# robertteleng/aria-slam

Measured on AMD Instinct MI355X. Metric: frames/s ORB extract+BF-match, 640x480 @2000 kp, higher is better.
Workload: dtype u8

## Files before the change

aria_slam_amd/csrc/orb_kernels.h:

```cpp
#pragma once
#include <hip/hip_runtime.h>
#include <hip/hip_ext.h>

#include <cstdint>
#include <vector>

#include "aria_orb_hip.h"
#include "orb_plan.h"

namespace aria {

struct FrameSrc {
    const uint8_t* img;
    int64_t frame_stride;
    int row_stride;
    int aligned4;
    int aligned16;
};

struct DeviceScratch {
    uint8_t* raw;
    uint8_t* blur;
    uint32_t* cand;
    int* cand_cnt;
    uint4* sel;
    int* sel_cnt;
    uint32_t* tab;
    int* pyr_bands;
    int* err;
    int* ovf;
    int2* ovf_items;
    unsigned long long* ovf_keys;
    long long ovf_keys_cap;
    uint4* osel;
    int osel_cap;
};

enum { STAGE_RESIZE = 0, STAGE_FAST_BLUR = 1, STAGE_SELECT = 2, STAGE_DESCRIBE = 3, STAGE_COUNT = 4 };
struct LaunchEvents { hipEvent_t start, stop; int stage; int launches; };
struct Profiler {
    bool enabled = false;
    unsigned stage_mask = ~0u;
    bool open = false;
    std::vector<LaunchEvents> pending;
    std::vector<hipEvent_t> pool;
    double ms[STAGE_COUNT] = {0, 0, 0, 0};
    int64_t launches[STAGE_COUNT] = {0, 0, 0, 0};
    int64_t frames = 0;
    LaunchEvents cur{};
    hipEvent_t get();
    void begin(int stage, hipStream_t st);
    void count() { cur.launches++; }
    void end(hipStream_t st);
    void collect();
    void release();
};

struct EnvConfig {
    int ablate;
    int level_streams;
    int stamp_level;
    int sel_stamps;
    int band_trim;
    int band_xcd_map;
    int select_bitonic;
    int desc_stamps;
    int fast_blur_impl;
    int fuse_resize;
    int pyr_impl;
    int rs_impl;
    int band_budget_kb, band_qpct0, band_qstep;
    int batch_stream;
};
const EnvConfig& env_config();

struct LaunchCtx {
    int device = -1;
    int schedule = 0;
    int* hdr = nullptr;
    const uint8_t* host_img = nullptr;
    hipEvent_t stage_event[4] = {};
    bool stage_events_armed = false;
    bool last_blur_q4 = false;
    const char* last_fast_blur = "";
    hipStream_t side[kLevels] = {};
    hipEvent_t ev_fork = nullptr, ev_join[kLevels] = {}, ev_lvl[kLevels] = {};
    unsigned long long* d_band_stamps = nullptr;
    unsigned long long* d_sel_stamps = nullptr;
    unsigned long long* d_desc_stamps = nullptr;
    int init(int device);
    void release();
};

#define ARIA_LAUNCH(prof, kernel, grid, block, lds, st, ...)                       \
    do {                                                                           \
        if ((prof) && (prof)->open) (prof)->count();                               \
        hipLaunchKernelGGL(kernel, grid, block, lds, st, __VA_ARGS__);             \
    } while (0)

void launch_fast_blur_band(const Plan& P, const FrameSrc& S, const DeviceScratch& D, int n_frames, hipStream_t st,
                           Profiler* prof, bool fuse_resize, LaunchCtx& ctx);
void launch_band2(const Plan& P, const FrameSrc& S, const DeviceScratch& D, int n_frames, hipStream_t st, Profiler* prof,
                  bool fuse_resize, LaunchCtx& ctx);
int band2_set_attributes();
void launch_fast_blur_stream(const Plan& P, const FrameSrc& S, const DeviceScratch& D, int n_frames, hipStream_t st,
                             Profiler* prof, LaunchCtx& ctx);
bool stream_eligible(const Plan& P, const FrameSrc& S);
int stream_set_attributes();
int blur_tail_start(int tie_mode, int w);
int band_set_attributes();
int band_init_ctx(LaunchCtx& ctx);
int band_side_streams(LaunchCtx& ctx);

struct BandAll { int first[kLevels + 1]; int qcap[kLevels]; int xcd_map; int lpr[kLevels]; };
bool launch_pyramid_fused(const Plan& P, const FrameSrc& S, const DeviceScratch& D, int n_frames, hipStream_t st, Profiler* prof,
                          int* clr_a = nullptr, int n_a = 0, int* clr_b = nullptr, int n_b = 0,
                          const uint8_t* src_alt = nullptr, uint8_t* copy_dst = nullptr);
bool pyramid_fused_available(const Plan& P);
bool latency_zero_copy(const Plan& P, const LaunchCtx& ctx, const Profiler* prof);
void launch_pyramid_level(const Plan& P, const FrameSrc& S, const DeviceScratch& D, int n_frames, hipStream_t st, Profiler* prof, int l);
void launch_pyramid_and_band_latency(const Plan& P, const FrameSrc& S, const DeviceScratch& D, int n_frames, hipStream_t st,
                                     Profiler* prof, LaunchCtx& ctx);
void launch_pyramid_pass(const Plan& P, const FrameSrc& S, const DeviceScratch& D, int n_frames, hipStream_t st, Profiler* prof);
int pyramid_set_attributes();
void launch_fast_blur_tile(const Plan& P, const FrameSrc& S, const DeviceScratch& D, int n_frames, hipStream_t st, Profiler* prof);

void launch_extract_chunk(const Plan& P, const FrameSrc& S, const DeviceScratch& D, int n_frames,
                          aria_keypoint* d_kps, uint8_t* d_desc, int* d_counts, int kp_cap, hipStream_t st,
                          Profiler* prof, LaunchCtx& ctx);

}
```

aria_slam_amd/csrc/orb_kernels.hip:

```cpp
#include <hip/hip_runtime.h>

#include <cfloat>
#include <cstdint>
#include <cstdlib>

#include "common.h"
#include "orb_device.h"
#include "orb_kernels.h"

namespace aria {

struct PatternLaneMajor { uint32_t w[16][16]; };
constexpr PatternLaneMajor make_pattern_lane_major() {
    constexpr int src[1024] = {
#include "orb_pattern_31.inc"
    };
    PatternLaneMajor p{};
    for (int l = 0; l < 16; l++)
        for (int it = 0; it < 16; it++) {
            const int t = 16 * it + l;
            p.w[l][it] = ((uint32_t)(src[4 * t] & 0xFF)) | ((uint32_t)(src[4 * t + 1] & 0xFF) << 8) |
                         ((uint32_t)(src[4 * t + 2] & 0xFF) << 16) | ((uint32_t)(src[4 * t + 3] & 0xFF) << 24);
        }
    return p;
// ... 470 lines not shown
                uint32_t u = __float_as_uint(r);
                u = (u & 0x80000000u) ? ~u : (u | 0x80000000u);
                key = ((unsigned long long)(~u) << 32) | ((uint32_t)y << 16) | (uint32_t)x;
            }
            const unsigned long long m = __ballot(keep);
            if (m) {
                const int lane = tid & 63, leader = __ffsll((long long)m) - 1;
                int base = 0;
                if (lane == leader) base = atomicAdd(&s_misc[1], __popcll(m));
                base = __shfl(base, leader);
                if (keep) ovf_st(&K[base + __popcll(m & ((1ull << lane) - 1ull))], key);
            }
        }
        for (long long i = n1 + tid; i < np; i += 256) ovf_st(&K[i], ~0ull);
        __syncthreads();
        for (long long k = 2; k <= np; k <<= 1)
            for (long long j = k >> 1; j > 0; j >>= 1) {
                for (long long t = tid; t < (np >> 1); t += 256) {
                    const long long a = ((t & ~(j - 1)) << 1) | (t & (j - 1)), b = a | j;
                    const unsigned long long xa = ovf_ld(&K[a]), xb = ovf_ld(&K[b]);
                    if ((xa > xb) == ((a & k) == 0)) { ovf_st(&K[a], xb); ovf_st(&K[b], xa); }
                }
                __syncthreads();
            }
        int n2 = n1;
        if (n1 > q) {
            const uint32_t cut = (uint32_t)(ovf_ld(&K[q - 1]) >> 32);
            for (int i = q + tid; i < n1; i += 256)
                if ((uint32_t)(ovf_ld(&K[i]) >> 32) == cut) atomicAdd(&s_misc[2], 1);
            __syncthreads();
            n2 = q + s_misc[2];
        }
        const int extra = max(n2 - g.sel_cap, 0), extra4 = (extra + 3) & ~3;
        if (tid == 0) {
            int ob = 0;
            if (extra4 > 0) {
                ob = atomicAdd(&ovf[1], extra4);
                if (ob + extra4 > osel_cap) { atomicOr(err, ERRBIT_SEL_OVERFLOW); ob = -1; }
            }
            s_misc[4] = ob;
        }
        __syncthreads();
        const int ob = s_misc[4];
        if (ob < 0) n2 = g.sel_cap;
        uint4* out = sel + (int64_t)frame * P.sel_frame_entries + g.sel_off;
        const uint32_t tag = (uint32_t)frame | ((uint32_t)l << 24);
        for (int i = tid; i < n2; i += 256) {
            const unsigned long long kk = ovf_ld(&K[i]);
            uint32_t u = ~(uint32_t)(kk >> 32);
            u = (u & 0x80000000u) ? (u & 0x7FFFFFFFu) : ~u;
            const uint4 rec = make_uint4((uint32_t)kk, u, (uint32_t)i, tag);
            if (i < g.sel_cap) out[i] = rec;
            else osel[ob + (i - g.sel_cap)] = rec;
        }
        if (ob >= 0)
            for (int i = extra + tid; i < extra4; i += 256) osel[ob + i] = make_uint4(0u, 0u, 0xFFFFFFFFu, tag);
        if (tid == 0) sel_cnt[frame * kLevels + l] = n2;
    }
}

__global__ __launch_bounds__(256) void k_select_ovf(Plan P, FrameSrc S, const uint8_t* __restrict__ raw,
                                                    const uint32_t* __restrict__ cand, const int* __restrict__ cand_cnt,
                                                    uint4* __restrict__ sel, int* __restrict__ sel_cnt, int* __restrict__ err,
                                                    int* __restrict__ ovf, const int2* __restrict__ ovf_items,
                                                    unsigned long long* __restrict__ keys, long long keys_cap,
                                                    uint4* __restrict__ osel, int osel_cap) {
    __shared__ int s_hist[256];
    __shared__ __attribute__((aligned(8))) int s_misc[8];
    const int n_items = min(ovf[0], kOvfItems);
    for (int it = blockIdx.x; it < n_items; it += gridDim.x)
        select_ovf_item(P, S, raw, cand, cand_cnt, sel, sel_cnt, err, ovf, keys, keys_cap, osel, osel_cap, ovf_items[it].x,
                        ovf_items[it].y, s_hist, s_misc);
}

__device__ __forceinline__ float fast_atan2_deg(float y, float x) {
    const float p1 = 0.9997878412794807f * (float)(180 / 3.1415926535897932384626433832795);
    const float p3 = -0.3258083974640975f * (float)(180 / 3.1415926535897932384626433832795);
    const float p5 = 0.1555786518463281f * (float)(180 / 3.1415926535897932384626433832795);
    const float p7 = -0.04432655554792128f * (float)(180 / 3.1415926535897932384626433832795);
    const float ax = fabsf(x), ay = fabsf(y);
    float a, c, c2;
    if (ax >= ay) {
        c = ay / (ax + (float)DBL_EPSILON);
        c2 = c * c;
        a = (((p7 * c2 + p5) * c2 + p3) * c2 + p1) * c;
    } else {
        c = ax / (ay + (float)DBL_EPSILON);
        c2 = c * c;
        a = 90.f - (((p7 * c2 + p5) * c2 + p3) * c2 + p1) * c;
    }
    if (x < 0) a = 180.f - a;
    if (y < 0) a = 360.f - a;
    return a;
}

__device__ __forceinline__ void det_sincos(double x, double& s, double& c) {
    const double invpio2 = 6.36619772367581382433e-01;
    const double pio2_hi = 1.57079632673412561417e+00;
    const double pio2_lo = 6.07710050650619224932e-11;
    const double S1 = -1.66666666666666324348e-01, S2 = 8.33333333332248946124e-03,
                 S3 = -1.98412698298579493134e-04, S4 = 2.75573137070700676789e-06,
                 S5 = -2.50507602534068634195e-08, S6 = 1.58969099521155010221e-10;
    const double C1 = 4.16666666666666019037e-02, C2 = -1.38888888888741095749e-03,
                 C3 = 2.48015872894767294178e-05, C4 = -2.75573143513906633035e-07,
                 C5 = 2.08757232129817482790e-09, C6 = -1.13596475577881948265e-11;
    const double fn = floor(x * invpio2 + 0.5);
    const double r = (x - fn * pio2_hi) - fn * pio2_lo;
    const double z = r * r;
    const double sp = S2 + z * (S3 + z * (S4 + z * (S5 + z * S6)));
    const double sn = r + (z * r) * (S1 + z * sp);
    const double cp = z * (C1 + z * (C2 + z * (C3 + z * (C4 + z * (C5 + z * C6)))));
    const double cs = 1.0 - (0.5 * z - z * cp);
    const int qd = (int)fn & 3;
    s = (qd == 0) ? sn : (qd == 1) ? cs : (qd == 2) ? -sn : -cs;
    c = (qd == 0) ? cs : (qd == 1) ? -sn : (qd == 2) ? -cs : sn;
}

__device__ __forceinline__ int wave_sum(int v) {
    v += __builtin_amdgcn_update_dpp(0, v, 0xB1, 0xF, 0xF, true);
    v += __builtin_amdgcn_update_dpp(0, v, 0x4E, 0xF, 0xF, true);
    v += __builtin_amdgcn_update_dpp(0, v, 0x141, 0xF, 0xF, true);
    v += __builtin_amdgcn_update_dpp(0, v, 0x140, 0xF, 0xF, true);
    v += __builtin_amdgcn_update_dpp(0, v, 0x142, 0xA, 0xF, false);
    v += __builtin_amdgcn_update_dpp(0, v, 0x143, 0xC, 0xF, false);
    return __builtin_amdgcn_readlane(v, 63);
}

constexpr int kDescR = 18;
constexpr int kDescRows = 2 * kDescR + 1;
constexpr int kDescPitch = 64;
constexpr int kDescWaves = 2;
constexpr int kDescKp = 4 * kDescWaves;
constexpr int kIcPitch = 48;
struct __attribute__((packed, aligned(4))) DwordQuad { uint32_t a, b, c, d; };

__device__ __forceinline__ int row8_sum(int v) {
    v += __builtin_amdgcn_update_dpp(0, v, 0xB1, 0xF, 0xF, true);
    v += __builtin_amdgcn_update_dpp(0, v, 0x4E, 0xF, 0xF, true);
    v += __builtin_amdgcn_update_dpp(0, v, 0x141, 0xF, 0xF, true);
    return v;
}

__device__ __forceinline__ int row16_sum(int v) {
    v += __builtin_amdgcn_update_dpp(0, v, 0xB1, 0xF, 0xF, true);
    v += __builtin_amdgcn_update_dpp(0, v, 0x4E, 0xF, 0xF, true);
    v += __builtin_amdgcn_update_dpp(0, v, 0x141, 0xF, 0xF, true);
    v += __builtin_amdgcn_update_dpp(0, v, 0x140, 0xF, 0xF, true);
    return v;
}

constexpr int kDescArenaBlocks = 32;
constexpr int kDescQ = 10;
constexpr int kDescPitchQ = 4 * kDescQ;
template <int MODE, bool Q4>
__global__ __launch_bounds__(64 * kDescWaves) void k_describe(Plan P, FrameSrc S, const uint8_t* __restrict__ raw,
                                                  const uint8_t* __restrict__ blur, const uint4* __restrict__ sel,
                                                  const int* __restrict__ sel_cnt, aria_keypoint* __restrict__ kps,
                                                  uint8_t* __restrict__ desc, int* __restrict__ counts, int kp_cap,
                                                  int* __restrict__ err, int n_frames, int blocks_per_frame,
                                                  unsigned long long* __restrict__ stamps,
                                                  const uint4* __restrict__ osel, const int* __restrict__ ovf, int osel_cap) {
#define DSTAMP(k) do { if (stamps && (threadIdx.x & 63) == 0) stamps[((size_t)blockIdx.x * kDescWaves + (threadIdx.x >> 6)) * 8 + (k)] = __builtin_amdgcn_s_memtime(); } while (0)
    DSTAMP(0);
    constexpr int kPatchBytes = Q4 ? kDescPitchQ * kDescPitchQ : kDescRows * kDescPitch;
    static_assert(kPatchBytes >= 31 * kIcPitch && kPatchBytes % 16 == 0, "the raw window shares the allocation");
    __shared__ __attribute__((aligned(16))) uint8_t s_patch[kDescKp][kPatchBytes];
    uint8_t (*s_raw)[kPatchBytes] = s_patch;
    const int lane = threadIdx.x & 63, wv = threadIdx.x >> 6;
    const int grp = lane >> 4, l16 = lane & 15;
    const int n_regular = MODE == 2 ? (int)gridDim.x - kDescArenaBlocks : (int)gridDim.x;
    auto describe_block = [&](const int blk_in, const bool ARENA) {
    const int blk = __builtin_amdgcn_readfirstlane(blk_in);
    int frame, l = 0, base = 0, nk;
    uint4 sv;
    if (!ARENA) {
        const int xcd = blk & 7, j = blk >> 3;
        frame = __builtin_amdgcn_readfirstlane((j / blocks_per_frame) * 8 + xcd);
        if (frame >= n_frames) return;
        const int jm = __builtin_amdgcn_readfirstlane(j % blocks_per_frame);
        const int slot0 = __builtin_amdgcn_readfirstlane(jm * kDescKp + wv * 4);
        const int* cnt = sel_cnt + frame * kLevels;
        int total = 0;
#pragma unroll
        for (int i = 0; i < kLevels; i++) {
            const int ci = cnt[i];
            if (i > 0 && slot0 >= P.lv[i].sel_off) { l = i; base = total; }
            total += ci;
        }
        if (slot0 == 0 && lane == 0) {
            counts[frame] = min(total, kp_cap);
            if (total > kp_cap) atomicMax(err + 2, total);
        }
        if (slot0 >= P.sel_frame_entries) return;
        l = __builtin_amdgcn_readfirstlane(l);
        base = __builtin_amdgcn_readfirstlane(base);
        const int i0 = slot0 - P.lv[l].sel_off;
        nk = min(4, min(cnt[l], P.lv[l].sel_cap) - i0);
        if (nk <= 0) return;
        sv = sel[(int64_t)frame * P.sel_frame_entries + slot0 + min(grp, nk - 1)];
    } else {
        const int e0 = blk * kDescKp + wv * 4;
        if (e0 >= min(ovf[1], osel_cap)) return;
        const uint4 mine = osel[e0 + grp];
        const unsigned long long vm = __ballot(mine.z != 0xFFFFFFFFu && l16 == 0);
        nk = __popcll(vm);
        if (nk <= 0) return;
        const uint32_t tag = (uint32_t)__builtin_amdgcn_readfirstlane((int)mine.w);
        frame = (int)(tag & 0xFFFFFFu);
        l = (int)(tag >> 24);
        const int* cnt = sel_cnt + frame * kLevels;
        for (int i = 0; i < l; i++) base += cnt[i];
        sv = osel[e0 + min(grp, nk - 1)];
    }
    const LevelGeom g = P.lv[l];
    const bool valid = grp < nk;
    const int oidx = base + (int)sv.z;
    const bool fits = oidx < kp_cap;
    if (valid && !fits && l16 == 0) atomicOr(err, ERRBIT_KPCAP);
    const int x = sv.x & 0xFFFF, y = sv.x >> 16;
    if (stamps) { asm volatile("s_waitcnt vmcnt(0)" ::: "memory"); }
    DSTAMP(1);

    uint32_t icm[16];
#pragma unroll
    for (int k = 0; k < 16; k += 4) {
        const uint4 m4 = *reinterpret_cast<const uint4*>(&kIcMask.m[l16][k]);
        icm[k] = m4.x; icm[k + 1] = m4.y; icm[k + 2] = m4.z; icm[k + 3] = m4.w;
    }
    int pat[16];
#pragma unroll
    for (int it = 0; it < 16; it += 4) {
        const uint4 p4 = *reinterpret_cast<const uint4*>(&kPattern31.w[l16][it]);
        pat[it] = (int)p4.x; pat[it + 1] = (int)p4.y; pat[it + 2] = (int)p4.z; pat[it + 3] = (int)p4.w;
    }

    const uint8_t* bl = blur + (int64_t)frame * P.blur_frame_bytes + g.blur_off;
    const int xs = Q4 ? ((x - kDescR) & ~3) : ((x - kDescR) & ~15);
    const int ys = Q4 ? ((y - kDescR) & ~3) : (y - kDescR);
    constexpr int kPv = Q4 ? 7 : 10;
    DwordQuad pv[kPv];
    int pq[kPv], pc[kPv];
    if constexpr (Q4) {
        const int64_t qp = (int64_t)g.pitch * 4;
        const uint8_t* gp = bl + (int64_t)(ys >> 2) * qp + (xs >> 2) * 16;
#pragma unroll
        for (int k = 0; k < kPv; k++) {
            const int p = min(16 * k + l16, kDescQ * kDescQ - 1);
            pq[k] = (p * 205) >> 11;
            pc[k] = p - kDescQ * pq[k];
            pv[k] = *reinterpret_cast<const DwordQuad*>(gp + pq[k] * qp + pc[k] * 16);
        }
    } else {
        const int r4 = l16 >> 2, c4 = l16 & 3;
        const int64_t p64 = g.pitch;
        const uint8_t* gp = bl + (int64_t)(y - kDescR) * p64 + xs + 16 * c4;
#pragma unroll
        for (int k = 0; k < 10; k++) {
            const int row = (4 * k + 4 <= kDescRows) ? 4 * k + r4 : min(4 * k + r4, kDescRows - 1);
            pv[k] = *reinterpret_cast<const DwordQuad*>(gp + row * p64);
        }
        (void)pq; (void)pc;
    }
    const int rr = l16 / 3, cc = l16 - 3 * rr;
    int pitch;
    const uint8_t* img = raw_level_ptr(P, S, raw, frame, l, pitch);
    const bool raw_dword = __builtin_amdgcn_readfirstlane((l > 0) || S.aligned4) != 0;
    const bool raw_a16 = __builtin_amdgcn_readfirstlane((l > 0) || S.aligned16) != 0;
    const int xr = raw_a16 ? ((x - kHalfPatch) & ~15) : ((x - kHalfPatch) & ~3);
    {
        uint8_t* sr = s_raw[wv * 4 + grp] + 16 * cc;
        const int64_t p64 = pitch;
        const uint8_t* gp = img + (int64_t)(y - kHalfPatch) * p64 + xr + 16 * cc;
        DwordQuad rv[7];
        if (raw_dword) {
#pragma unroll
            for (int k = 0; k < 7; k++) {
                const int row = (5 * k + 5 < 31) ? 5 * k + rr : min(5 * k + rr, 30);
                rv[k] = *reinterpret_cast<const DwordQuad*>(gp + row * p64);
            }
        } else {
#pragma unroll
            for (int k = 0; k < 7; k++) {
                const int row = (5 * k + 5 < 31) ? 5 * k + rr : min(5 * k + rr, 30);
                const uint8_t* q = gp + row * p64;
                rv[k].a = (uint32_t)q[0] | ((uint32_t)q[1] << 8) | ((uint32_t)q[2] << 16) | ((uint32_t)q[3] << 24);
                rv[k].b = (uint32_t)q[4] | ((uint32_t)q[5] << 8) | ((uint32_t)q[6] << 16) | ((uint32_t)q[7] << 24);
                rv[k].c = (uint32_t)q[8] | ((uint32_t)q[9] << 8) | ((uint32_t)q[10] << 16) | ((uint32_t)q[11] << 24);
                rv[k].d = (uint32_t)q[12] | ((uint32_t)q[13] << 8) | ((uint32_t)q[14] << 16) | ((uint32_t)q[15] << 24);
            }
        }
#pragma unroll
        for (int k = 0; k < 7; k++) {
            const int row = (5 * k + 5 < 31) ? 5 * k + rr : min(5 * k + rr, 30);
            *reinterpret_cast<uint4*>(sr + row * kIcPitch) = make_uint4(rv[k].a, rv[k].b, rv[k].c, rv[k].d);
        }
    }
    if (stamps) { asm volatile("s_waitcnt vmcnt(0) lgkmcnt(0)" ::: "memory"); }
    DSTAMP(2);
    __builtin_amdgcn_wave_barrier();

    const int sh = (x - xr) - kHalfPatch;
    const int hp = l16 >> 3, jj = l16 & 7;
    const uint8_t* rbase = s_raw[wv * 4 + grp] + 4 * jj + (sh & ~3);
    const uint32_t wu = 0x04030201u + 0x04040404u * (uint32_t)jj;
    uint32_t acc_u = 0, acc_v = 0, acc_s = 0;
#pragma unroll
    for (int k = 0; k < 16; k++) {
        const int r = min(2 * k + hp, 30);
        const uint32_t lo = *reinterpret_cast<const uint32_t*>(rbase + r * kIcPitch);
        const uint32_t hi = *reinterpret_cast<const uint32_t*>(rbase + r * kIcPitch + 4);
        const uint32_t pix = __builtin_amdgcn_alignbyte(hi, lo, sh) & icm[k];
        acc_u = __builtin_amdgcn_udot4(pix, wu, acc_u, false);
        acc_v = __builtin_amdgcn_udot4(pix, 0x01010101u * (uint32_t)(2 * k + 1), acc_v, false);
        acc_s = __builtin_amdgcn_sad_u8(pix, 0u, acc_s);
    }
    const int sum_u = row16_sum((int)acc_u), sum_v = row16_sum((int)acc_v);
    const int s_half = row8_sum((int)acc_s);
    const int s_othr = __builtin_amdgcn_update_dpp(0, s_half, 0x140, 0xF, 0xF, true);
    const int s_all = s_half + s_othr;
    const int s_hp1 = hp ? s_half : s_othr;
    const int m10 = sum_u - 16 * s_all;
    const int m01 = sum_v + s_hp1 - 16 * s_all;
    const float angle = fast_atan2_deg((float)m01, (float)m10);
    DSTAMP(3);

    float ang = angle;
    ang *= (float)(3.1415926535897932384626433832795 / 180.f);
    double sd, cd;
    det_sincos((double)ang, sd, cd);
    const float a = (float)cd, b = (float)sd;
    __builtin_amdgcn_wave_barrier();
    constexpr int kPitchL = Q4 ? kDescPitchQ : kDescPitch;
    if constexpr (Q4) {
        uint8_t* sp = s_patch[wv * 4 + grp];
#pragma unroll
        for (int k = 0; k < kPv; k++) {
            uint32_t* d = reinterpret_cast<uint32_t*>(sp + (4 * pq[k]) * kPitchL + 4 * pc[k]);
            d[0] = pv[k].a; d[kPitchL / 4] = pv[k].b; d[2 * kPitchL / 4] = pv[k].c; d[3 * kPitchL / 4] = pv[k].d;
        }
    } else {
        const int r4 = l16 >> 2, c4 = l16 & 3;
        uint8_t* sp = s_patch[wv * 4 + grp] + 16 * c4;
#pragma unroll
        for (int k = 0; k < 10; k++) {
            const int row = (4 * k + 4 <= kDescRows) ? 4 * k + r4 : min(4 * k + r4, kDescRows - 1);
            *reinterpret_cast<uint4*>(sp + row * kDescPitch) = make_uint4(pv[k].a, pv[k].b, pv[k].c, pv[k].d);
        }
    }
    const uint8_t* bc = s_patch[wv * 4 + grp] + (y - ys) * kPitchL + (x - xs);
    __builtin_amdgcn_wave_barrier();
    typedef float f2 __attribute__((ext_vector_type(2)));
    const f2 aa = {a, a}, bb = {b, b}, nbb = {-b, -b};
    const f2 magic = {12582912.0f, 12582912.0f};
    constexpr uint32_t kMagicBits = 0x4B400000u;
    const uint8_t* bc0 = bc - (size_t)(0x400000u * (uint32_t)kPitchL + kMagicBits);
    DSTAMP(4);
    uint32_t mine = 0;
#pragma unroll
    for (int it = 0; it < 16; it++) {
        const float px0 = (float)(signed char)(pat[it] & 0xFF), py0 = (float)(signed char)((pat[it] >> 8) & 0xFF);
        const float px1 = (float)(signed char)((pat[it] >> 16) & 0xFF), py1 = (float)(signed char)((pat[it] >> 24) & 0xFF);
        const f2 PX = {px0, px1}, PY = {py0, py1};
        const f2 fx = PX * aa + PY * nbb + magic;
        const f2 fy = PX * bb + PY * aa + magic;
        const uint32_t o0 = __umul24(__float_as_uint(fy.x), kPitchL) + __float_as_uint(fx.x);
        const uint32_t o1 = __umul24(__float_as_uint(fy.y), kPitchL) + __float_as_uint(fx.y);
        const int t0 = bc0[o0];
        const int t1 = bc0[o1];
        const unsigned long long m = __ballot(t0 < t1);
        if (__builtin_amdgcn_inverse_ballot_w64(0x0001000100010001ull << it)) mine = (uint32_t)(m >> (16 * grp)) & 0xFFFFu;
    }
    DSTAMP(5);
    if (valid && fits) {
        const int64_t orow = (int64_t)frame * kp_cap + oidx;
        *reinterpret_cast<uint16_t*>(desc + orow * 32 + 2 * l16) = (uint16_t)mine;
        if (l16 == 0) {
            aria_keypoint k;
            k.x = (float)x * g.scale;
            k.y = (float)y * g.scale;
            k.size = kPatchSize * g.scale;
            k.angle = angle;
            k.response = __uint_as_float(sv.y);
            k.octave = l;
            kps[orow] = k;
        }
    }
    };
    if constexpr (MODE == 0) {
        describe_block((int)blockIdx.x, false);
    } else if constexpr (MODE == 1) {
        const int n_blk = (min(ovf[1], osel_cap) + kDescKp - 1) / kDescKp;
        for (int blk = blockIdx.x; blk < n_blk; blk += gridDim.x) describe_block(blk, true);
    } else {
        if ((int)blockIdx.x < n_regular) {
            describe_block((int)blockIdx.x, false);
        } else {
            const int n_blk = (min(ovf[1], osel_cap) + kDescKp - 1) / kDescKp;
            for (int blk = (int)blockIdx.x - n_regular; blk < n_blk; blk += kDescArenaBlocks) describe_block(blk, true);
        }
    }
    DSTAMP(6);
#undef DSTAMP
}

static int env_int(const char* name, int dflt) { const char* e = aria_getenv(name); return e ? atoi(e) : dflt; }
static bool env_is(const char* name, char c) { const char* e = aria_getenv(name); return e && e[0] == c; }

const EnvConfig& env_config() {
    static const EnvConfig cfg = [] {
        EnvConfig c{};
        c.ablate = env_int("ARIA_ABLATE", 0);
        c.level_streams = env_is("ARIA_LEVEL_STREAMS", '1') ? 1 : 0;
        c.stamp_level = env_int("ARIA_STAMPS", -1);
        c.sel_stamps = env_is("ARIA_SEL_STAMPS", '1') ? 1 : 0;
        c.select_bitonic = env_is("ARIA_SELECT_SORT", 'b') ? 1 : 0;
        c.band_xcd_map = env_is("ARIA_BAND_XCD_MAP", '0') ? 0 : 1;
        c.band_trim = env_is("ARIA_BAND_TRIM", '0') ? 0 : 1;
        c.desc_stamps = env_is("ARIA_DESC_STAMPS", '1') ? 1 : 0;
        c.fast_blur_impl = env_is("ARIA_FAST_BLUR_IMPL", 't') ? 0 : env_is("ARIA_FAST_BLUR_IMPL", 'm') ? 1 : 2;
        c.pyr_impl = env_is("ARIA_PYRAMID_IMPL", 'f') ? 1 : 0;
        c.rs_impl = env_is("ARIA_RESIZE_IMPL", 'd') ? 0 : env_is("ARIA_RESIZE_IMPL", 'l') ? 1 : 2;
        c.fuse_resize = (c.fast_blur_impl != 0 && !env_is("ARIA_RESIZE_FUSE", '0') && !aria_getenv("ARIA_RESIZE_IMPL") &&
                         !aria_getenv("ARIA_PYRAMID_IMPL") && !c.level_streams) ? 1 : 0;
        c.band_budget_kb = env_int("ARIA_BAND_BUDGET_KB", 0);
        c.band_qpct0 = env_int("ARIA_BAND_QPCT0", -1);
        c.band_qstep = env_int("ARIA_BAND_QPCT_STEP", -1);
        c.batch_stream = (c.fast_blur_impl == 2 && !env_is("ARIA_FAST_BLUR_IMPL", 'b') && c.fuse_resize && c.stamp_level < 0) ? 1 : 0;
        return c;
    }();
    return cfg;
}

hipEvent_t Profiler::get() {
    if (!pool.empty()) { hipEvent_t e = pool.back(); pool.pop_back(); return e; }
    hipEvent_t e = nullptr;
    if (hipEventCreate(&e) != hipSuccess) return nullptr;
    return e;
}
void Profiler::begin(int stage, hipStream_t st) {
    open = enabled && ((stage_mask >> stage) & 1u);
    if (!open) return;
    cur = LaunchEvents{get(), get(), stage, 0};
    hipStreamSynchronize(st);
    hipEventRecord(cur.start, st);
}
void Profiler::end(hipStream_t st) {
    if (!open) return;
    open = false;
    hipEventRecord(cur.stop, st);
    hipStreamSynchronize(st);
    pending.push_back(cur);
}
void Profiler::collect() {
    for (LaunchEvents& le : pending) {
        float t = 0.f;
        if (hipEventElapsedTime(&t, le.start, le.stop) == hipSuccess) ms[le.stage] += t;
        launches[le.stage] += le.launches;
        pool.push_back(le.start);
        pool.push_back(le.stop);
    }
    pending.clear();
}
void Profiler::release() {
    collect();
    for (hipEvent_t e : pool) hipEventDestroy(e);
    pool.clear();
}

int LaunchCtx::init(int dev) {
    device = dev;
    const EnvConfig& E = env_config();
    ARIA_HIP(hipFuncSetAttribute(reinterpret_cast<const void*>(k_select<false, 256>), hipFuncAttributeMaxDynamicSharedMemorySize,
                                 (int)(sizeof(unsigned long long) * kSortCapMax)));
    ARIA_HIP(hipFuncSetAttribute(reinterpret_cast<const void*>(k_select<true, 256>), hipFuncAttributeMaxDynamicSharedMemorySize,
                                 (int)(sizeof(unsigned long long) * kSortCapMax)));
    if (int prc = pyramid_set_attributes(); prc != ARIA_OK) return prc;
    int rc = band_set_attributes();
    if (rc != ARIA_OK) return rc;
#ifdef ARIA_VARIANTS
    rc = band2_set_attributes();
    if (rc != ARIA_OK) return rc;
#endif
    rc = stream_set_attributes();
    if (rc != ARIA_OK) return rc;
    rc = band_init_ctx(*this);
    if (rc != ARIA_OK) return rc;
    if (E.sel_stamps) ARIA_HIP(hipMalloc(&d_sel_stamps, sizeof(unsigned long long) * 8 * kLevels * 4096));
    if (E.desc_stamps) ARIA_HIP(hipMalloc(&d_desc_stamps, sizeof(unsigned long long) * 8 * (1u << 22)));
    return ARIA_OK;
}

void LaunchCtx::release() {
    for (int l = 0; l < kLevels; l++) {
        if (side[l]) hipStreamDestroy(side[l]);
        if (ev_join[l]) hipEventDestroy(ev_join[l]);
        if (ev_lvl[l]) hipEventDestroy(ev_lvl[l]);
        side[l] = nullptr; ev_join[l] = nullptr; ev_lvl[l] = nullptr;
    }
    if (ev_fork) hipEventDestroy(ev_fork);
    ev_fork = nullptr;
    hipFree(d_band_stamps); hipFree(d_sel_stamps); hipFree(d_desc_stamps);
    d_band_stamps = d_sel_stamps = d_desc_stamps = nullptr;
}

static bool latency_schedule(const LaunchCtx& ctx, const Profiler* prof) {
    return ctx.schedule == 1 && ctx.ev_fork != nullptr && env_config().fast_blur_impl == 2 && !(prof && prof->enabled);
}

bool latency_zero_copy(const Plan& P, const LaunchCtx& ctx, const Profiler* prof) {
    static const bool off = [] { const char* e = aria_getenv("ARIA_ZERO_COPY"); return !(e && e[0] == '1'); }();
    const char* f = aria_getenv("ARIA_LATENCY_FORK");
    return !off && !(f && f[0] == '1') && ctx.host_img != nullptr && latency_schedule(ctx, prof) && pyramid_fused_available(P);
}

void launch_extract_chunk(const Plan& P, const FrameSrc& S, const DeviceScratch& D, int n_frames,
                          aria_keypoint* d_kps, uint8_t* d_desc, int* d_counts, int kp_cap, hipStream_t st,
                          Profiler* prof, LaunchCtx& ctx) {
    const EnvConfig& E = env_config();
    if (prof && prof->enabled) prof->frames += n_frames;

    const bool latency = latency_schedule(ctx, prof);
    const bool fuse_resize = E.fuse_resize != 0 && !latency;
    ctx.last_blur_q4 = false;
    if (!latency) {
        hipMemsetAsync(D.ovf, 0, sizeof(int) * (4 + kLevels * (size_t)n_frames), st);
        if (ctx.hdr) hipMemsetAsync(ctx.hdr, 0, 64, st);
    }
    if (latency) {
        ctx.last_fast_blur = "k_fast_blur_band";
        launch_pyramid_and_band_latency(P, S, D, n_frames, st, prof, ctx);
    } else {
#ifdef ARIA_VARIANTS
    if (!fuse_resize) {
        if (prof) prof->begin(STAGE_RESIZE, st);
        launch_pyramid_pass(P, S, D, n_frames, st, prof);
        if (prof) prof->end(st);
    }
#endif

    if (prof) prof->begin(STAGE_FAST_BLUR, st);
    if (E.batch_stream && fuse_resize && stream_eligible(P, S)) {
        ctx.last_fast_blur = "k_fast_blur_stream";
        ctx.last_blur_q4 = true;
        launch_fast_blur_stream(P, S, D, n_frames, st, prof, ctx);
#ifdef ARIA_VARIANTS
    } else if (E.fast_blur_impl == 1 && !E.level_streams && P.tie_mode <= 1) {
        ctx.last_fast_blur = "k_band2";
        launch_band2(P, S, D, n_frames, st, prof, fuse_resize, ctx);
    } else if (E.fast_blur_impl == 0 && P.tie_mode <= 1) {
        ctx.last_fast_blur = "k_fast_blur";
        launch_fast_blur_tile(P, S, D, n_frames, st, prof);
#endif
    } else {
        ctx.last_fast_blur = "k_fast_blur_band";
        launch_fast_blur_band(P, S, D, n_frames, st, prof, fuse_resize, ctx);
    }
    if (prof) prof->end(st);
    }

    if (ctx.stage_events_armed && ctx.stage_event[STAGE_SELECT]) hipEventRecord(ctx.stage_event[STAGE_SELECT], st);
    if (prof) prof->begin(STAGE_SELECT, st);
    unsigned long long* sstp = (ctx.d_sel_stamps && n_frames <= 4096) ? ctx.d_sel_stamps : nullptr;
    if (sstp) hipMemsetAsync(sstp, 0, sizeof(unsigned long long) * 8 * kLevels * (size_t)n_frames, st);
    if (latency)
        ARIA_LAUNCH(prof, (k_select<true, 256>), dim3(kLevels, n_frames), dim3(256), sizeof(unsigned long long) * (size_t)P.sort_cap,
                    st, P, S, D.raw, D.cand, D.cand_cnt, D.sel, D.sel_cnt, D.err, sstp, D.ovf, D.ovf_items, D.ovf_keys,
                    D.ovf_keys_cap, D.osel, D.osel_cap, E.select_bitonic);
    else
        ARIA_LAUNCH(prof, (k_select<false, 256>), dim3(kLevels, n_frames), dim3(256), sizeof(unsigned long long) * (size_t)P.sort_cap,
                    st, P, S, D.raw, D.cand, D.cand_cnt, D.sel, D.sel_cnt, D.err, sstp, D.ovf, D.ovf_items, D.ovf_keys,
                    D.ovf_keys_cap, D.osel, D.osel_cap, E.select_bitonic);
    if (!latency)
    ARIA_LAUNCH(prof, k_select_ovf, dim3(64), dim3(256), 0, st, P, S, D.raw, D.cand, D.cand_cnt, D.sel, D.sel_cnt, D.err,
                D.ovf, D.ovf_items, D.ovf_keys, D.ovf_keys_cap, D.osel, D.osel_cap);
    if (sstp) {
        hipStreamSynchronize(st);
        std::vector<unsigned long long> hs((size_t)n_frames * kLevels * 8);
        hipMemcpy(hs.data(), sstp, hs.size() * 8, hipMemcpyDeviceToHost);
        for (int l = 0; l < kLevels; l += 7) {
            double ph[5] = {0}; int n = 0;
            for (int f = 0; f < n_frames; f++) {
                const unsigned long long* q = &hs[((size_t)f * kLevels + l) * 8];
                if (!q[5]) continue;
                for (int k = 0; k < 5; k++) ph[k] += (double)(q[k + 1] - q[k]);
                n++;
            }
            if (n) fprintf(stderr, "[select stamps L%d] %d blocks, cycles: hist %.0f cut+compact %.0f harris %.0f sort %.0f emit %.0f\n",
                           l, n, ph[0] / n, ph[1] / n, ph[2] / n, ph[3] / n, ph[4] / n);
        }
    }

    if (prof) prof->end(st);

    if (prof) prof->begin(STAGE_DESCRIBE, st);
    {
        const int bpf = (P.sel_frame_entries + kDescKp - 1) / kDescKp;
        const int frames8 = (n_frames + 7) / 8 * 8;
        const size_t nwaves = (size_t)bpf * frames8 * kDescWaves;
        unsigned long long* stp = (ctx.d_desc_stamps && nwaves <= (1u << 22)) ? ctx.d_desc_stamps : nullptr;
        if (stp) hipMemsetAsync(stp, 0, sizeof(unsigned long long) * 8 * nwaves, st);
        if (latency) {
            ARIA_LAUNCH(prof, (k_describe<2, false>), dim3((unsigned)(bpf * frames8 + kDescArenaBlocks)), dim3(64 * kDescWaves), 0, st, P, S,
                        D.raw, D.blur, D.sel, D.sel_cnt, d_kps, d_desc, d_counts, kp_cap, D.err, n_frames, bpf, stp,
                        (const uint4*)D.osel, (const int*)D.ovf, D.osel_cap);
        } else if (ctx.last_blur_q4) {
            ARIA_LAUNCH(prof, (k_describe<0, true>), dim3((unsigned)(bpf * frames8)), dim3(64 * kDescWaves), 0, st, P, S, D.raw, D.blur,
                        D.sel, D.sel_cnt, d_kps, d_desc, d_counts, kp_cap, D.err, n_frames, bpf, stp, (const uint4*)nullptr,
                        (const int*)nullptr, 0);
            ARIA_LAUNCH(prof, (k_describe<1, true>), dim3(256), dim3(64 * kDescWaves), 0, st, P, S,
                        D.raw, D.blur, D.sel, D.sel_cnt, d_kps, d_desc, d_counts, kp_cap, D.err, n_frames, bpf,
                        (unsigned long long*)nullptr, (const uint4*)D.osel, (const int*)D.ovf, D.osel_cap);
        } else {
            ARIA_LAUNCH(prof, (k_describe<0, false>), dim3((unsigned)(bpf * frames8)), dim3(64 * kDescWaves), 0, st, P, S, D.raw, D.blur,
                        D.sel, D.sel_cnt, d_kps, d_desc, d_counts, kp_cap, D.err, n_frames, bpf, stp, (const uint4*)nullptr,
                        (const int*)nullptr, 0);
            ARIA_LAUNCH(prof, (k_describe<1, false>), dim3(256), dim3(64 * kDescWaves), 0, st, P, S,
                        D.raw, D.blur, D.sel, D.sel_cnt, d_kps, d_desc, d_counts, kp_cap, D.err, n_frames, bpf,
                        (unsigned long long*)nullptr, (const uint4*)D.osel, (const int*)D.ovf, D.osel_cap);
        }
        if (stp) {
            hipStreamSynchronize(st);
            std::vector<unsigned long long> hs(nwaves * 8);
            hipMemcpy(hs.data(), stp, hs.size() * 8, hipMemcpyDeviceToHost);
            double ph[6] = {0}; size_t n = 0;
            for (size_t w = 0; w < nwaves; w++) {
                if (!hs[w * 8 + 6] || !hs[w * 8 + 5] || !hs[w * 8 + 1]) continue;
                for (int k = 0; k < 6; k++) ph[k] += (double)(hs[w * 8 + k + 1] - hs[w * 8 + k]);
                n++;
            }
            if (n) fprintf(stderr, "[describe stamps] %zu waves, 100 MHz ticks: sel %.1f windows %.1f moments+atan %.1f sincos %.1f pattern %.1f store %.1f\n",
                           n, ph[0] / n, ph[1] / n, ph[2] / n, ph[3] / n, ph[4] / n, ph[5] / n);
        }
    }
    if (prof) prof->end(st);
}

}
```

Before: 381,100.

## Add 16-keypoint-per-wave describe kernel for batch Q4 path and make it default

```diff
diff --git a/aria_slam_amd/csrc/orb_kernels.h b/aria_slam_amd/csrc/orb_kernels.h
--- a/aria_slam_amd/csrc/orb_kernels.h
+++ b/aria_slam_amd/csrc/orb_kernels.h
@@ -65,6 +65,7 @@
     int band_xcd_map;
     int select_bitonic;
     int desc_stamps;
+    int desc_quad;
     int fast_blur_impl;
     int fuse_resize;
     int pyr_impl;
diff --git a/aria_slam_amd/csrc/orb_kernels.hip b/aria_slam_amd/csrc/orb_kernels.hip
--- a/aria_slam_amd/csrc/orb_kernels.hip
+++ b/aria_slam_amd/csrc/orb_kernels.hip
@@ -646,14 +646,328 @@
 constexpr int kDescArenaBlocks = 32;
 constexpr int kDescQ = 10;
 constexpr int kDescPitchQ = 4 * kDescQ;
-template <int MODE, bool Q4>
-__global__ __launch_bounds__(64 * kDescWaves) void k_describe(Plan P, FrameSrc S, const uint8_t* __restrict__ raw,
+
+constexpr int kDesc16Kp = 16;
+__device__ __forceinline__ int row_src(int r) { return (((int)(threadIdx.x & 0x30)) | r) << 2; }
+__device__ __forceinline__ int row_pick(int v, int src) { return __builtin_amdgcn_ds_bpermute(src, v); }
+
+__host__ __device__ __forceinline__ int desc16_waves_per_frame(const Plan& P) {
+    int w = 0;
+    for (int i = 0; i < kLevels; i++) w += (P.lv[i].sel_cap + kDesc16Kp - 1) / kDesc16Kp;
+    return w;
+}
+
+template <int MODE>
+__device__ __forceinline__ void describe16(const Plan& P, const FrameSrc& S, const uint8_t* __restrict__ raw,
+                                           const uint8_t* __restrict__ blur, const uint4* __restrict__ sel,
+                                           const int* __restrict__ sel_cnt, aria_keypoint* __restrict__ kps,
+                                           uint8_t* __restrict__ desc, int* __restrict__ counts, int kp_cap,
+                                           int* __restrict__ err, int n_frames, int blocks_per_frame,
+                                           unsigned long long* __restrict__ stamps,
+                                           const uint4* __restrict__ osel, const int* __restrict__ ovf, int osel_cap,
+                                           const int blk_in) {
+    constexpr bool ARENA = MODE == 1;
+#define DSTAMP16(k) do { if (stamps && (threadIdx.x & 63) == 0) stamps[((size_t)blockIdx.x * kDescWaves + (threadIdx.x >> 6)) * 8 + (k)] = __builtin_amdgcn_s_memtime(); } while (0)
+    DSTAMP16(0);
+    constexpr int kPatchBytes = kDescPitchQ * kDescPitchQ;
+    static_assert(kPatchBytes >= 31 * kIcPitch && kPatchBytes % 16 == 0, "the raw window shares the allocation");
+    __shared__ __attribute__((aligned(16))) uint8_t s_patch[kDescKp][kPatchBytes];
+    const int lane = threadIdx.x & 63, wv = threadIdx.x >> 6;
+    const int grp = lane >> 4, l16 = lane & 15;
+    const int rs = l16 & 3;
+    uint8_t* const win = s_patch[wv * 4 + grp];
+
+    int frame = 0, l = 0, base = 0;
+    uint4 sv;
+    bool valid;
+    uint32_t act = 0;
+    if constexpr (!ARENA) {
+        const int blk = __builtin_amdgcn_readfirstlane(blk_in);
+        const int xcd = blk & 7, j = blk >> 3;
+        frame = __builtin_amdgcn_readfirstlane((j / blocks_per_frame) * 8 + xcd);
+        if (frame >= n_frames) return;
+        const int w = __builtin_amdgcn_readfirstlane((j % blocks_per_frame) * kDescWaves + wv);
+        const int* cnt = sel_cnt + frame * kLevels;
+        int total = 0, wl = 0, i0 = -1;
+#pragma unroll
+        for (int i = 0; i < kLevels; i++) {
+            const int ci = cnt[i];
+            const int nw = (P.lv[i].sel_cap + kDesc16Kp - 1) / kDesc16Kp;
+            if (w >= wl && w < wl + nw) { l = i; base = total; i0 = kDesc16Kp * (w - wl); }
+            wl += nw;
+            total += ci;
+        }
+        if (w == 0 && lane == 0) {
+            counts[frame] = min(total, kp_cap);
+            if (total > kp_cap) atomicMax(err + 2, total);
+        }
+        if (i0 < 0) return;
+        l = __builtin_amdgcn_readfirstlane(l);
+        base = __builtin_amdgcn_readfirstlane(base);
+        const int nk = min(kDesc16Kp, min(cnt[l], P.lv[l].sel_cap) - i0);
+        if (nk <= 0) return;
+        act = (1u << ((nk + 3) >> 2)) - 1u;
+        const int k = 4 * rs + grp;
+        valid = l16 < 4 && k < nk;
+        sv = sel[(int64_t)frame * P.sel_frame_entries + P.lv[l].sel_off + i0 + min(k, nk - 1)];
+    } else {
+        const int e0 = __builtin_amdgcn_readfirstlane((blk_in * kDescWaves + wv) * kDesc16Kp);
+        const int n_arena = min(ovf[1], osel_cap);
+        if (e0 >= n_arena) return;
+        const bool blk_ok = e0 + 4 * rs < n_arena;
+        const int eb = e0 + 4 * rs;
+        const bool live = blk_ok && osel[eb + grp].z != 0xFFFFFFFFu;
+        const unsigned long long vm = __ballot(live && l16 < 4);
+        const int nkr = __popcll(vm & (0x0001000100010001ull << rs));
+        valid = l16 < 4 && grp < nkr;
+#pragma unroll
+        for (int r = 0; r < 4; r++)
+            if ((vm & (0x0001000100010001ull << r)) && act == (1u << r) - 1u) act |= 1u << r;
+        if (act == 0) return;
+        sv = blk_ok ? osel[eb + min(grp, max(nkr, 1) - 1)] : make_uint4(0u, 0u, 0u, 0u);
+    }
+    auto round_fl = [&](int r, int& fr, int& lr) {
+        if constexpr (ARENA) {
+            const uint32_t tag = (uint32_t)__builtin_amdgcn_readlane((int)sv.w, r);
+            fr = (int)(tag & 0xFFFFFFu);
+            lr = (int)(tag >> 24);
+        } else {
+            fr = frame; lr = l;
+        }
+    };
+    const int x_s = sv.x & 0xFFFF, y_s = sv.x >> 16;
+    if (stamps) { asm volatile("s_waitcnt vmcnt(0)" ::: "memory"); }
+    DSTAMP16(1);
+
+    uint32_t icm[16];
+#pragma unroll
+    for (int k = 0; k < 16; k += 4) {
+        const uint4 m4 = *reinterpret_cast<const uint4*>(&kIcMask.m[l16][k]);
+        icm[k] = m4.x; icm[k + 1] = m4.y; icm[k + 2] = m4.z; icm[k + 3] = m4.w;
+    }
+    const int rr = l16 / 3, cc = l16 - 3 * rr;
+    const int hp = l16 >> 3, jj = l16 & 7;
+    const uint32_t wu = 0x04030201u + 0x04040404u * (uint32_t)jj;
+    DwordQuad rv[7];
+    int sh_n = 0;
+    auto raw_issue = [&](int r) {
+        int fr, lr;
+        round_fl(r, fr, lr);
+        int pitch;
+        const uint8_t* img = raw_level_ptr(P, S, raw, fr, lr, pitch);
+        const bool raw_dword = __builtin_amdgcn_readfirstlane((lr > 0) || S.aligned4) != 0;
+        const bool raw_a16 = __builtin_amdgcn_readfirstlane((lr > 0) || S.aligned16) != 0;
+        const int xy = row_pick((int)sv.x, row_src(r));
+        const int x = xy & 0xFFFF, y = (int)((uint32_t)xy >> 16);
+        const int xr = raw_a16 ? ((x - kHalfPatch) & ~15) : ((x - kHalfPatch) & ~3);
+        sh_n = (x - xr) - kHalfPatch;
+        const uint32_t o = (uint32_t)((y - kHalfPatch) * pitch + xr + 16 * cc);
+        if (raw_dword) {
+#pragma unroll
+            for (int k = 0; k < 7; k++) {
+                const int row = (5 * k + 5 < 31) ? 5 * k + rr : min(5 * k + rr, 30);
+                rv[k] = *reinterpret_cast<const DwordQuad*>(img + (o + (uint32_t)(row * pitch)));
+            }
+        } else {
+#pragma unroll
+            for (int k = 0; k < 7; k++) {
+                const int row = (5 * k + 5 < 31) ? 5 * k + rr : min(5 * k + rr, 30);
+                const uint8_t* q = img + (o + (uint32_t)(row * pitch));
+                rv[k].a = (uint32_t)q[0] | ((uint32_t)q[1] << 8) | ((uint32_t)q[2] << 16) | ((uint32_t)q[3] << 24);
+                rv[k].b = (uint32_t)q[4] | ((uint32_t)q[5] << 8) | ((uint32_t)q[6] << 16) | ((uint32_t)q[7] << 24);
+                rv[k].c = (uint32_t)q[8] | ((uint32_t)q[9] << 8) | ((uint32_t)q[10] << 16) | ((uint32_t)q[11] << 24);
+                rv[k].d = (uint32_t)q[12] | ((uint32_t)q[13] << 8) | ((uint32_t)q[14] << 16) | ((uint32_t)q[15] << 24);
+            }
+        }
+    };
+    constexpr int kPv = 7;
+    DwordQuad pv[kPv];
+    int pq[kPv], pc[kPv];
+#pragma unroll
+    for (int k = 0; k < kPv; k++) {
+        const int p = min(16 * k + l16, kDescQ * kDescQ - 1);
+        pq[k] = (p * 205) >> 11;
+        pc[k] = p - kDescQ * pq[k];
+    }
+    auto blur_issue = [&](int r) {
+        int fr, lr;
+        round_fl(r, fr, lr);
+        const uint8_t* bl = blur + (int64_t)fr * P.blur_frame_bytes + P.lv[lr].blur_off;
+        const int qp = P.lv[lr].pitch * 4;
+        const int xy = row_pick((int)sv.x, row_src(r));
+        const int x = xy & 0xFFFF, y = (int)((uint32_t)xy >> 16);
+        const uint32_t o = (uint32_t)(((y - kDescR) >> 2) * qp + ((x - kDescR) >> 2) * 16);
+#pragma unroll
+        for (int k = 0; k < kPv; k++)
+            pv[k] = *reinterpret_cast<const DwordQuad*>(bl + (o + (uint32_t)(pq[k] * qp + pc[k] * 16)));
+    };
+
+    int m10_s = 0, m01_s = 0;
+    const int nr = 32 - __builtin_clz(act);
+    auto moment_round = [&](int r, auto next) {
+        const int sh = sh_n;
+        {
+            uint8_t* sr = win + 16 * cc;
+#pragma unroll
+            for (int k = 0; k < 7; k++) {
+                const int row = (5 * k + 5 < 31) ? 5 * k + rr : min(5 * k + rr, 30);
+                *reinterpret_cast<uint4*>(sr + row * kIcPitch) = make_uint4(rv[k].a, rv[k].b, rv[k].c, rv[k].d);
+            }
+        }
+        next();
+        __builtin_amdgcn_wave_barrier();
+        const uint8_t* rbase = win + 4 * jj + (sh & ~3);
+        uint32_t acc_u = 0, acc_v = 0, acc_s = 0;
+#pragma unroll
+        for (int k = 0; k < 16; k++) {
+            const int rw = min(2 * k + hp, 30);
+            const uint32_t lo = *reinterpret_cast<const uint32_t*>(rbase + rw * kIcPitch);
+            const uint32_t hi = *reinterpret_cast<const uint32_t*>(rbase + rw * kIcPitch + 4);
+            const uint32_t pix = __builtin_amdgcn_alignbyte(hi, lo, sh) & icm[k];
+            acc_u = __builtin_amdgcn_udot4(pix, wu, acc_u, false);
+            acc_v = __builtin_amdgcn_udot4(pix, 0x01010101u * (uint32_t)(2 * k + 1), acc_v, false);
+            acc_s = __builtin_amdgcn_sad_u8(pix, 0u, acc_s);
+        }
+        const int sum_u = row16_sum((int)acc_u), sum_v = row16_sum((int)acc_v);
+        const int s_half = row8_sum((int)acc_s);
+        const int s_othr = __builtin_amdgcn_update_dpp(0, s_half, 0x140, 0xF, 0xF, true);
+        const int s_all = s_half + s_othr;
+        const int s_hp1 = hp ? s_half : s_othr;
+        if (l16 == r) {
+            m10_s = sum_u - 16 * s_all;
+            m01_s = sum_v + s_hp1 - 16 * s_all;
+        }
+        __builtin_amdgcn_wave_barrier();
+    };
+    raw_issue(0);
+#pragma unroll 1
+    for (int r = 0; r < nr - 1; r++) moment_round(r, [&] { raw_issue(r + 1); });
+    moment_round(nr - 1, [&] { blur_issue(0); });
+    if (stamps) { asm volatile("s_waitcnt vmcnt(0) lgkmcnt(0)" ::: "memory"); }
+    DSTAMP16(2);
+
+    const float angle_s = fast_atan2_deg((float)m01_s, (float)m10_s);
+    float ang = angle_s;
+    ang *= (float)(3.1415926535897932384626433832795 / 180.f);
+    double sd, cd;
+    det_sincos((double)ang, sd, cd);
+    const float a_s = (float)cd, b_s = (float)sd;
+    int base_s = base, frame_s = frame, l_s = l;
+    if constexpr (ARENA) {
+        const uint32_t tag = sv.w;
+        frame_s = (int)(tag & 0xFFFFFFu);
+        l_s = (int)(tag >> 24);
+        base_s = 0;
+        if (valid) {
+            const int* cnt = sel_cnt + frame_s * kLevels;
+            for (int i = 0; i < l_s; i++) base_s += cnt[i];
+        }
+    }
+    const int oidx_s = base_s + (int)sv.z;
+    const bool fits_s = oidx_s < kp_cap;
+    if (valid && !fits_s) atomicOr(err, ERRBIT_KPCAP);
+    const int orow_s = (valid && fits_s) ? oidx_s : -1;
+    if (stamps) { asm volatile("s_waitcnt vmcnt(0) lgkmcnt(0)" ::: "memory"); }
+    DSTAMP16(3);
+
+    int pat[16];
+#pragma unroll
+    for (int it = 0; it < 16; it += 4) {
+        const uint4 p4 = *reinterpret_cast<const uint4*>(&kPattern31.w[l16][it]);
+        pat[it] = (int)p4.x; pat[it + 1] = (int)p4.y; pat[it + 2] = (int)p4.z; pat[it + 3] = (int)p4.w;
+    }
+    typedef float f2 __attribute__((ext_vector_type(2)));
+    const f2 magic = {12582912.0f, 12582912.0f};
+    constexpr uint32_t kMagicBits = 0x4B400000u;
+    constexpr int kPitchL = kDescPitchQ;
+#pragma unroll 1
+    for (int r = 0; r < nr; r++) {
+        const int src = row_src(r);
+        const int xy = row_pick((int)sv.x, src);
+        const int x = xy & 0xFFFF, y = (int)((uint32_t)xy >> 16);
+        const int xs = (x - kDescR) & ~3, ys = (y - kDescR) & ~3;
+        const float a = __int_as_float(row_pick(__float_as_int(a_s), src));
+        const float b = __int_as_float(row_pick(__float_as_int(b_s), src));
+        const int orow = row_pick(orow_s, src);
+        __builtin_amdgcn_wave_barrier();
+#pragma unroll
+        for (int k = 0; k < kPv; k++) {
+            uint32_t* d = reinterpret_cast<uint32_t*>(win + (4 * pq[k]) * kPitchL + 4 * pc[k]);
+            d[0] = pv[k].a; d[kPitchL / 4] = pv[k].b; d[2 * kPitchL / 4] = pv[k].c; d[3 * kPitchL / 4] = pv[k].d;
+        }
+        if (r + 1 < nr) blur_issue(r + 1);
+        const uint8_t* bc = win + (y - ys) * kPitchL + (x - xs);
+        __builtin_amdgcn_wave_barrier();
+        const f2 aa = {a, a}, bb = {b, b}, nbb = {-b, -b};
+        const uint8_t* bc0 = bc - (size_t)(0x400000u * (uint32_t)kPitchL + kMagicBits);
+#pragma unroll
+        for (int it = 0; it < 16; it++) asm volatile("" : "+v"(pat[it]));
+        uint32_t mine = 0;
+#pragma unroll
+        for (int it = 0; it < 16; it++) {
+            const float px0 = (float)(signed char)(pat[it] & 0xFF), py0 = (float)(signed char)((pat[it] >> 8) & 0xFF);
+            const float px1 = (float)(signed char)((pat[it] >> 16) & 0xFF), py1 = (float)(signed char)((pat[it] >> 24) & 0xFF);
+            const f2 PX = {px0, px1}, PY = {py0, py1};
+            const f2 fx = PX * aa + PY * nbb + magic;
+            const f2 fy = PX * bb + PY * aa + magic;
+            const uint32_t o0 = __umul24(__float_as_uint(fy.x), kPitchL) + __float_as_uint(fx.x);
+            const uint32_t o1 = __umul24(__float_as_uint(fy.y), kPitchL) + __float_as_uint(fx.y);
+            const int t0 = bc0[o0];
+            const int t1 = bc0[o1];
+            const unsigned long long m = __ballot(t0 < t1);
+            if (__builtin_amdgcn_inverse_ballot_w64(0x0001000100010001ull << it)) mine = (uint32_t)(m >> (16 * grp)) & 0xFFFFu;
+        }
+        if (orow >= 0) {
+            int fr, lr;
+            round_fl(r, fr, lr);
+            *reinterpret_cast<uint16_t*>(desc + ((int64_t)fr * kp_cap + orow) * 32 + 2 * l16) = (uint16_t)mine;
+        }
+        __builtin_amdgcn_wave_barrier();
+    }
+    if (stamps) { asm volatile("s_waitcnt vmcnt(0) lgkmcnt(0)" ::: "memory"); }
+    DSTAMP16(4);
+
+    if (orow_s >= 0) {
+        float scale = P.lv[l].scale;
+        if constexpr (ARENA) {
+#pragma unroll
+            for (int i = 1; i < kLevels; i++)
+                if (l_s == i) scale = P.lv[i].scale;
+        }
+        aria_keypoint k;
+        k.x = (float)x_s * scale;
+        k.y = (float)y_s * scale;
+        k.size = kPatchSize * scale;
+        k.angle = angle_s;
+        k.response = __uint_as_float(sv.y);
+        k.octave = l_s;
+        kps[(int64_t)frame_s * kp_cap + orow_s] = k;
+    }
+    DSTAMP16(5);
+#undef DSTAMP16
+}
+
+template <int MODE, bool Q4, bool W16 = false>
+__global__ __launch_bounds__(64 * kDescWaves, W16 && MODE == 0 ? 4 : 1) void k_describe(Plan P, FrameSrc S, const uint8_t* __restrict__ raw,
                                                   const uint8_t* __restrict__ blur, const uint4* __restrict__ sel,
                                                   const int* __restrict__ sel_cnt, aria_keypoint* __restrict__ kps,
                                                   uint8_t* __restrict__ desc, int* __restrict__ counts, int kp_cap,
                                                   int* __restrict__ err, int n_frames, int blocks_per_frame,
                                                   unsigned long long* __restrict__ stamps,
                                                   const uint4* __restrict__ osel, const int* __restrict__ ovf, int osel_cap) {
+    if constexpr (W16) {
+        static_assert(Q4 && MODE < 2, "the 16-keypoint form is the batch Q4 form");
+        if constexpr (MODE == 0) {
+            describe16<0>(P, S, raw, blur, sel, sel_cnt, kps, desc, counts, kp_cap, err, n_frames, blocks_per_frame, stamps,
+                          osel, ovf, osel_cap, (int)blockIdx.x);
+        } else {
+            const int n_blk = (min(ovf[1], osel_cap) + kDescWaves * kDesc16Kp - 1) / (kDescWaves * kDesc16Kp);
+            for (int blk = blockIdx.x; blk < n_blk; blk += gridDim.x)
+                describe16<1>(P, S, raw, blur, sel, sel_cnt, kps, desc, counts, kp_cap, err, n_frames, blocks_per_frame,
+                              stamps, osel, ovf, osel_cap, blk);
+        }
+        return;
+    }
 #define DSTAMP(k) do { if (stamps && (threadIdx.x & 63) == 0) stamps[((size_t)blockIdx.x * kDescWaves + (threadIdx.x >> 6)) * 8 + (k)] = __builtin_amdgcn_s_memtime(); } while (0)
     DSTAMP(0);
     constexpr int kPatchBytes = Q4 ? kDescPitchQ * kDescPitchQ : kDescRows * kDescPitch;
@@ -911,6 +1225,7 @@
         c.band_xcd_map = env_is("ARIA_BAND_XCD_MAP", '0') ? 0 : 1;
         c.band_trim = env_is("ARIA_BAND_TRIM", '0') ? 0 : 1;
         c.desc_stamps = env_is("ARIA_DESC_STAMPS", '1') ? 1 : 0;
+        c.desc_quad = env_is("ARIA_DESC_IMPL", 'q') ? 1 : 0;
         c.fast_blur_impl = env_is("ARIA_FAST_BLUR_IMPL", 't') ? 0 : env_is("ARIA_FAST_BLUR_IMPL", 'm') ? 1 : 2;
         c.pyr_impl = env_is("ARIA_PYRAMID_IMPL", 'f') ? 1 : 0;
         c.rs_impl = env_is("ARIA_RESIZE_IMPL", 'd') ? 0 : env_is("ARIA_RESIZE_IMPL", 'l') ? 1 : 2;
@@ -1088,7 +1403,8 @@
 
     if (prof) prof->begin(STAGE_DESCRIBE, st);
     {
-        const int bpf = (P.sel_frame_entries + kDescKp - 1) / kDescKp;
+        const bool w16 = !latency && ctx.last_blur_q4 && !E.desc_quad;
+        const int bpf = w16 ? (desc16_waves_per_frame(P) + kDescWaves - 1) / kDescWaves : (P.sel_frame_entries + kDescKp - 1) / kDescKp;
         const int frames8 = (n_frames + 7) / 8 * 8;
         const size_t nwaves = (size_t)bpf * frames8 * kDescWaves;
         unsigned long long* stp = (ctx.d_desc_stamps && nwaves <= (1u << 22)) ? ctx.d_desc_stamps : nullptr;
@@ -1097,6 +1413,14 @@
             ARIA_LAUNCH(prof, (k_describe<2, false>), dim3((unsigned)(bpf * frames8 + kDescArenaBlocks)), dim3(64 * kDescWaves), 0, st, P, S,
                         D.raw, D.blur, D.sel, D.sel_cnt, d_kps, d_desc, d_counts, kp_cap, D.err, n_frames, bpf, stp,
                         (const uint4*)D.osel, (const int*)D.ovf, D.osel_cap);
+        } else if (w16) {
+            ARIA_LAUNCH(prof, (k_describe<0, true, true>), dim3((unsigned)(bpf * frames8)), dim3(64 * kDescWaves), 0, st, P, S, D.raw,
+                        D.blur, D.sel, D.sel_cnt, d_kps, d_desc, d_counts, kp_cap, D.err, n_frames, bpf, stp, (const uint4*)nullptr,
+                        (const int*)nullptr, 0);
+            ARIA_LAUNCH(prof, (k_describe<1, true, true>), dim3(256), dim3(64 * kDescWaves), 0, st, P, S,
+                        D.raw, D.blur, D.sel, D.sel_cnt, d_kps, d_desc, d_counts, kp_cap, D.err, n_frames, bpf,
+                        (unsigned long long*)nullptr, (const uint4*)D.osel, (const int*)D.ovf, D.osel_cap);
+#ifdef ARIA_VARIANTS
         } else if (ctx.last_blur_q4) {
             ARIA_LAUNCH(prof, (k_describe<0, true>), dim3((unsigned)(bpf * frames8)), dim3(64 * kDescWaves), 0, st, P, S, D.raw, D.blur,
                         D.sel, D.sel_cnt, d_kps, d_desc, d_counts, kp_cap, D.err, n_frames, bpf, stp, (const uint4*)nullptr,
@@ -1104,6 +1428,7 @@
             ARIA_LAUNCH(prof, (k_describe<1, true>), dim3(256), dim3(64 * kDescWaves), 0, st, P, S,
                         D.raw, D.blur, D.sel, D.sel_cnt, d_kps, d_desc, d_counts, kp_cap, D.err, n_frames, bpf,
                         (unsigned long long*)nullptr, (const uint4*)D.osel, (const int*)D.ovf, D.osel_cap);
+#endif
         } else {
             ARIA_LAUNCH(prof, (k_describe<0, false>), dim3((unsigned)(bpf * frames8)), dim3(64 * kDescWaves), 0, st, P, S, D.raw, D.blur,
                         D.sel, D.sel_cnt, d_kps, d_desc, d_counts, kp_cap, D.err, n_frames, bpf, stp, (const uint4*)nullptr,
@@ -1117,13 +1442,19 @@
             std::vector<unsigned long long> hs(nwaves * 8);
             hipMemcpy(hs.data(), stp, hs.size() * 8, hipMemcpyDeviceToHost);
             double ph[6] = {0}; size_t n = 0;
+            const int np = w16 ? 5 : 6;
             for (size_t w = 0; w < nwaves; w++) {
-                if (!hs[w * 8 + 6] || !hs[w * 8 + 5] || !hs[w * 8 + 1]) continue;
-                for (int k = 0; k < 6; k++) ph[k] += (double)(hs[w * 8 + k + 1] - hs[w * 8 + k]);
+                if (!hs[w * 8 + np] || !hs[w * 8 + 1]) continue;
+                if (!w16 && !hs[w * 8 + 5]) continue;
+                for (int k = 0; k < np; k++) ph[k] += (double)(hs[w * 8 + k + 1] - hs[w * 8 + k]);
                 n++;
             }
-            if (n) fprintf(stderr, "[describe stamps] %zu waves, 100 MHz ticks: sel %.1f windows %.1f moments+atan %.1f sincos %.1f pattern %.1f store %.1f\n",
-                           n, ph[0] / n, ph[1] / n, ph[2] / n, ph[3] / n, ph[4] / n, ph[5] / n);
+            if (n && w16)
+                fprintf(stderr, "[describe stamps] 16-kp form, %zu waves, 100 MHz ticks: sel %.1f moment rounds %.1f atan+sincos %.1f pattern rounds %.1f records %.1f\n",
+                        n, ph[0] / n, ph[1] / n, ph[2] / n, ph[3] / n, ph[4] / n);
+            else if (n)
+                fprintf(stderr, "[describe stamps] %zu waves, 100 MHz ticks: sel %.1f windows %.1f moments+atan %.1f sincos %.1f pattern %.1f store %.1f\n",
+                        n, ph[0] / n, ph[1] / n, ph[2] / n, ph[3] / n, ph[4] / n, ph[5] / n);
         }
     }
     if (prof) prof->end(st);
```

New measurement: 396,000, median of 6. +3.9%, better.
